# argmaxinc/WhisperKit

Measured on NVIDIA H100. Metric: RTFx (audio-sec/s) whisper-large-v3 greedy, higher is better.
Workload: dtype bf16

## Files before the change

whisperkit_b200/csrc/attention_wgmma.cu:

```cuda
#include <stdio.h>
#include <stdlib.h>

#include "common.cuh"
#include "kernels.h"
#include "wgmma.cuh"

namespace wk {

static constexpr int kFaThreads = 384;
static constexpr int kFaBM = 128;
static constexpr int kFaBN = 128;
static constexpr int kFaD = 64;
static constexpr int kFaTile = kFaBN * kFaD * 2;
static constexpr int kFaStages = 4;
static constexpr int kFaSmem = kFaTile  + 2 * kFaStages * kFaTile  + 1024  + 256 ;

struct FaParams {
    int T, H, dm, n_kv_tiles;
    float scale_log2e;
};

__device__ __forceinline__ float fa_ex2(float x) {
    float y;
    asm("ex2.approx.ftz.f32 %0, %1;" : "=f"(y) : "f"(x));
    return y;
}

template <typename T>
__global__ void __launch_bounds__(kFaThreads, 1)
encoder_attention_wgmma_kernel(const __grid_constant__ CUtensorMap tm_qkv, T* __restrict__ out, const FaParams p) {
    extern __shared__ __align__(1024) uint8_t smem_raw[];
    uint8_t* smem = reinterpret_cast<uint8_t*>((reinterpret_cast<uintptr_t>(smem_raw) + 1023) & ~uintptr_t(1023));
    uint8_t* sQ = smem;
    uint8_t* sK = sQ + kFaTile;
    uint8_t* sV = sK + kFaStages * kFaTile;
    uint64_t* bars = reinterpret_cast<uint64_t*>(sV + kFaStages * kFaTile);
    uint64_t* q_full = bars;
    uint64_t* k_full = bars + 1;
    uint64_t* k_empty = k_full + kFaStages;
    uint64_t* v_full = k_empty + kFaStages;
    uint64_t* v_empty = v_full + kFaStages;

    const int warp = threadIdx.x >> 5, lane = threadIdx.x & 31;
    const int bh = blockIdx.y;
    const int b = bh / p.H, h = bh % p.H;
    const int q0 = blockIdx.x * kFaBM;
    const int n = p.n_kv_tiles;

    if (warp == 0 && lane == 0) {
        tma_prefetch_desc(&tm_qkv);
        mbar_init(q_full, 1);
        for (int i = 0; i < kFaStages; ++i) {
            mbar_init(&k_full[i], 1); mbar_init(&k_empty[i], 8);
            mbar_init(&v_full[i], 1); mbar_init(&v_empty[i], 8);
        }
        fence_barrier_init();
    }
    __syncthreads();

    if (warp < 4) {
        asm volatile("setmaxnreg.dec.sync.aligned.u32 40;");
        if (warp == 0 && lane == 0) {
            mbar_expect_tx(q_full, kFaTile);
            tma_load_3d(sQ, &tm_qkv, q_full, h * kFaD, q0, b);
            for (int j = 0; j < n; ++j) {
                const int st = j % kFaStages;
                const uint32_t ph = (j / kFaStages) & 1;
                mbar_wait_bounded(&k_empty[st], ph ^ 1);
                mbar_expect_tx(&k_full[st], kFaTile);
                tma_load_3d(sK + st * kFaTile, &tm_qkv, &k_full[st], p.dm + h * kFaD, j * kFaBN, b);
                mbar_wait_bounded(&v_empty[st], ph ^ 1);
                mbar_expect_tx(&v_full[st], kFaTile);
                tma_load_3d(sV + st * kFaTile, &tm_qkv, &v_full[st], 2 * p.dm + h * kFaD, j * kFaBN, b);
            }
        }
        return;
    }

    asm volatile("setmaxnreg.inc.sync.aligned.u32 232;");
    const int cw = (warp >> 2) - 1;
    const int c_lo = 2 * (lane & 3);
    const float c = p.scale_log2e;
    const uint64_t qd = wgmma_desc_sw128(smem_u32(sQ + cw * 64 * 128));
    float o[32];
#pragma unroll
    for (int i = 0; i < 32; ++i) o[i] = 0.f;
    float m_run[2] = {-INFINITY, -INFINITY}, l_run[2] = {0.f, 0.f};

    mbar_wait_bounded(q_full, 0);
    for (int j = 0; j < n; ++j) {
        const int st = j % kFaStages;
        const uint32_t ph = (j / kFaStages) & 1;
        float s[64];
        mbar_wait_bounded(&k_full[st], ph);
        const uint64_t kd = wgmma_desc_sw128(smem_u32(sK + st * kFaTile));
        wgmma_fence();
#pragma unroll
        for (int k = 0; k < kFaD / 16; ++k) Wgmma<T, 128>::ss(s, qd + (uint64_t)(2 * k), kd + (uint64_t)(2 * k), k > 0 ? 1u : 0u);
        wgmma_commit();
        wgmma_wait<0>();
        __syncwarp();
        if (lane == 0) mbar_arrive(&k_empty[st]);

        const int valid = p.T - j * kFaBN;
        if (valid < kFaBN) {
#pragma unroll
            for (int jj = 0; jj < 16; ++jj)
#pragma unroll
                for (int e = 0; e < 4; ++e)
                    if (8 * jj + c_lo + (e & 1) >= valid) s[4 * jj + e] = -INFINITY;
        }
        uint32_t pa[8][4];
#pragma unroll
        for (int hf = 0; hf < 2; ++hf) {
            float mx = m_run[hf];
#pragma unroll
            for (int jj = 0; jj < 16; ++jj) mx = fmaxf(mx, fmaxf(s[4 * jj + 2 * hf], s[4 * jj + 2 * hf + 1]));
            mx = fmaxf(mx, __shfl_xor_sync(0xffffffffu, mx, 1));
            mx = fmaxf(mx, __shfl_xor_sync(0xffffffffu, mx, 2));
            const float corr = fa_ex2((m_run[hf] - mx) * c);
            m_run[hf] = mx;
            const float nmc = -mx * c;
            float sum = 0.f;
#pragma unroll
            for (int jj = 0; jj < 16; ++jj) {
                const float e0 = fa_ex2(fmaf(s[4 * jj + 2 * hf], c, nmc));
                const float e1 = fa_ex2(fmaf(s[4 * jj + 2 * hf + 1], c, nmc));
                sum += e0 + e1;
                pa[jj >> 1][(jj & 1) * 2 + hf] = T16<T>::pack2(e0, e1);
            }
            l_run[hf] = l_run[hf] * corr + sum;
#pragma unroll
            for (int jj = 0; jj < 8; ++jj) { o[4 * jj + 2 * hf] *= corr; o[4 * jj + 2 * hf + 1] *= corr; }
        }

        mbar_wait_bounded(&v_full[st], ph);
        const uint32_t vs = smem_u32(sV + st * kFaTile);
        wgmma_fence();
#pragma unroll
        for (int kk = 0; kk < kFaBN / 16; ++kk) Wgmma<T, 64>::rs_bt(o, pa[kk], wgmma_desc_sw128(vs + kk * 2048), 1u);
        wgmma_commit();
        wgmma_wait<0>();
        __syncwarp();
        if (lane == 0) mbar_arrive(&v_empty[st]);
    }

#pragma unroll
    for (int hf = 0; hf < 2; ++hf) {
        float l = l_run[hf];
        l += __shfl_xor_sync(0xffffffffu, l, 1);
        l += __shfl_xor_sync(0xffffffffu, l, 2);
        const float inv = 1.f / l;
        const int q = q0 + cw * 64 + (warp & 3) * 16 + (lane >> 2) + 8 * hf;
        if (q >= p.T) continue;
        T* dst = out + ((long long)b * p.T + q) * p.dm + h * kFaD + c_lo;
#pragma unroll
        for (int jj = 0; jj < 8; ++jj)
            *reinterpret_cast<uint32_t*>(dst + 8 * jj) = T16<T>::pack2(o[4 * jj + 2 * hf] * inv, o[4 * jj + 2 * hf + 1] * inv);
    }
}

typedef CUresult (*PFN_encodeTiled)(CUtensorMap*, CUtensorMapDataType, cuuint32_t, void*, const cuuint64_t*, const cuuint64_t*,
                                      const cuuint32_t*, const cuuint32_t*, CUtensorMapInterleave, CUtensorMapSwizzle,
                                      CUtensorMapL2promotion, CUtensorMapFloatOOBfill);

wk_status encoder_attention_wgmma(const void* qkv, void* out, int B, int T, int n_heads, int dtype, cudaStream_t stream) {
    static PFN_encodeTiled enc = nullptr;
    if (!enc) {
        void* fp = nullptr;
        cudaDriverEntryPointQueryResult q;
        if (cudaGetDriverEntryPoint("cuTensorMapEncodeTiled", &fp, cudaEnableDefault, &q) != cudaSuccess || q != cudaDriverEntryPointSuccess) {
            set_error("cuTensorMapEncodeTiled entry point unavailable");
            return WK_ERR_CUDA;
        }
        enc = reinterpret_cast<PFN_encodeTiled>(fp);
    }
    const int dm = n_heads * 64;
    CUtensorMap tm;
    cuuint64_t gdim[3] = {(cuuint64_t)3 * dm, (cuuint64_t)T, (cuuint64_t)B};
    cuuint64_t gstr[2] = {(cuuint64_t)3 * dm * 2, (cuuint64_t)T * 3 * dm * 2};
    cuuint32_t box[3] = {64, 128, 1};
    cuuint32_t es[3] = {1, 1, 1};
    CUresult r = enc(&tm, dtype == WK_DTYPE_F16 ? CU_TENSOR_MAP_DATA_TYPE_FLOAT16 : CU_TENSOR_MAP_DATA_TYPE_BFLOAT16, 3,
                     const_cast<void*>(qkv), gdim, gstr, box, es, CU_TENSOR_MAP_INTERLEAVE_NONE, CU_TENSOR_MAP_SWIZZLE_128B,
                     CU_TENSOR_MAP_L2_PROMOTION_L2_256B, CU_TENSOR_MAP_FLOAT_OOB_FILL_NONE);
    if (r != CUDA_SUCCESS) { set_error("attention tensor map encode failed: %d", (int)r); return WK_ERR_CUDA; }
    FaParams p;
    p.T = T; p.H = n_heads; p.dm = dm;
    p.n_kv_tiles = (T + kFaBN - 1) / kFaBN;
    p.scale_log2e = 0.125f * 1.4426950408889634f;
    dim3 grid((T + kFaBM - 1) / kFaBM, B * n_heads);
    cudaError_t e = cudaSuccess;
    if (dtype == WK_DTYPE_F16) {
        static bool set = false;
        if (!set) { e = cudaFuncSetAttribute(encoder_attention_wgmma_kernel<__half>, cudaFuncAttributeMaxDynamicSharedMemorySize, kFaSmem); set = e == cudaSuccess; }
        if (e == cudaSuccess) encoder_attention_wgmma_kernel<__half><<<grid, kFaThreads, kFaSmem, stream>>>(tm, (__half*)out, p);
    } else {
        static bool set = false;
        if (!set) { e = cudaFuncSetAttribute(encoder_attention_wgmma_kernel<__nv_bfloat16>, cudaFuncAttributeMaxDynamicSharedMemorySize, kFaSmem); set = e == cudaSuccess; }
        if (e == cudaSuccess) encoder_attention_wgmma_kernel<__nv_bfloat16><<<grid, kFaThreads, kFaSmem, stream>>>(tm, (__nv_bfloat16*)out, p);
    }
    if (e != cudaSuccess) { set_error("cudaFuncSetAttribute(fa): %s", cudaGetErrorString(e)); return WK_ERR_CUDA; }
    count_launch();
    e = cudaGetLastError();
    if (e != cudaSuccess) { set_error("encoder_attention_wgmma launch: %s", cudaGetErrorString(e)); return WK_ERR_CUDA; }
    return WK_OK;
}

}
```

Measured before the change: 919.8.

## Pipeline encoder attention: overlap QK^T with PV and ping-pong warpgroups

Restructures the consumer loop of the wgmma flash-attention kernel so that the S=QK^T GEMM for tile t is issued together with the PV GEMM for tile t-1, and softmax runs while the PV wgmma is still in flight. It also adds named-barrier turn-taking between the two consumer warpgroups so their tensor-core issue phases alternate with each other's softmax phases. The aim is to hide exponential and softmax latency behind tensor-core work. The cost is more live registers (s, pa and o held across iterations), extra named-barrier synchronisation, and more complex pipeline bookkeeping with prologue and epilogue stages.

Measured after the change: 927.8, median of 6. Within noise of the previous version (+0.9%).

```diff
diff --git a/whisperkit_b200/csrc/attention_wgmma.cu b/whisperkit_b200/csrc/attention_wgmma.cu
--- a/whisperkit_b200/csrc/attention_wgmma.cu
+++ b/whisperkit_b200/csrc/attention_wgmma.cu
@@ -20,10 +20,60 @@
     float scale_log2e;
 };
 
+struct FaSlot {
+    int st;
+    uint32_t ph;
+};
+__device__ __forceinline__ FaSlot fa_slot(int j) { return {j % kFaStages, (uint32_t)(j / kFaStages) & 1u}; }
+
+static constexpr int kFaTurnBar = 1;
+__device__ __forceinline__ void fa_turn_wait(int cw) { asm volatile("bar.sync %0, 256;" ::"r"(kFaTurnBar + cw) : "memory"); }
+__device__ __forceinline__ void fa_turn_pass(int cw) { asm volatile("bar.arrive %0, 256;" ::"r"(kFaTurnBar + (cw ^ 1)) : "memory"); }
+
+__device__ __forceinline__ void fa_wait(uint64_t* bar, uint32_t parity) {
+    if (mbar_try_wait(bar, parity)) return;
+    const unsigned long long t0 = globaltimer_ns();
+    unsigned int spins = 0;
+    while (!mbar_try_wait(bar, parity))
+        if ((++spins & 0xfffu) == 0 && globaltimer_ns() - t0 > kSpinLimitNs) __trap();
+}
+
 __device__ __forceinline__ float fa_ex2(float x) {
     float y;
     asm("ex2.approx.ftz.f32 %0, %1;" : "=f"(y) : "f"(x));
     return y;
+}
+
+__device__ __forceinline__ void fa_softmax(float (&s)[64], float (&m_run)[2], float (&l_run)[2], float (&corr)[2], int valid, int c_lo,
+                                           float c) {
+    if (valid < kFaBN) {
+#pragma unroll
+        for (int jj = 0; jj < 16; ++jj)
+#pragma unroll
+            for (int e = 0; e < 4; ++e)
+                if (8 * jj + c_lo + (e & 1) >= valid) s[4 * jj + e] = -INFINITY;
+    }
+#pragma unroll
+    for (int hf = 0; hf < 2; ++hf) {
+        float mx = m_run[hf];
+#pragma unroll
+        for (int jj = 0; jj < 16; ++jj) mx = fmaxf(mx, fmaxf(s[4 * jj + 2 * hf], s[4 * jj + 2 * hf + 1]));
+        mx = fmaxf(mx, __shfl_xor_sync(0xffffffffu, mx, 1));
+        mx = fmaxf(mx, __shfl_xor_sync(0xffffffffu, mx, 2));
+        corr[hf] = fa_ex2((m_run[hf] - mx) * c);
+        m_run[hf] = mx;
+        const float nmc = -mx * c;
+        float sum = 0.f;
+#pragma unroll
+        for (int jj = 0; jj < 16; ++jj) {
+            const float e0 = fa_ex2(fmaf(s[4 * jj + 2 * hf], c, nmc));
+            const float e1 = fa_ex2(fmaf(s[4 * jj + 2 * hf + 1], c, nmc));
+            sum += e0 + e1;
+            s[4 * jj + 2 * hf] = e0;
+            s[4 * jj + 2 * hf + 1] = e1;
+        }
+        l_run[hf] = l_run[hf] * corr[hf] + sum;
+    }
 }
 
 template <typename T>
@@ -64,14 +114,13 @@
             mbar_expect_tx(q_full, kFaTile);
             tma_load_3d(sQ, &tm_qkv, q_full, h * kFaD, q0, b);
             for (int j = 0; j < n; ++j) {
-                const int st = j % kFaStages;
-                const uint32_t ph = (j / kFaStages) & 1;
-                mbar_wait_bounded(&k_empty[st], ph ^ 1);
-                mbar_expect_tx(&k_full[st], kFaTile);
-                tma_load_3d(sK + st * kFaTile, &tm_qkv, &k_full[st], p.dm + h * kFaD, j * kFaBN, b);
-                mbar_wait_bounded(&v_empty[st], ph ^ 1);
-                mbar_expect_tx(&v_full[st], kFaTile);
-                tma_load_3d(sV + st * kFaTile, &tm_qkv, &v_full[st], 2 * p.dm + h * kFaD, j * kFaBN, b);
+                const FaSlot sl = fa_slot(j);
+                fa_wait(&k_empty[sl.st], sl.ph ^ 1);
+                mbar_expect_tx(&k_full[sl.st], kFaTile);
+                tma_load_3d(sK + sl.st * kFaTile, &tm_qkv, &k_full[sl.st], p.dm + h * kFaD, j * kFaBN, b);
+                fa_wait(&v_empty[sl.st], sl.ph ^ 1);
+                mbar_expect_tx(&v_full[sl.st], kFaTile);
+                tma_load_3d(sV + sl.st * kFaTile, &tm_qkv, &v_full[sl.st], 2 * p.dm + h * kFaD, j * kFaBN, b);
             }
         }
         return;
@@ -86,63 +135,81 @@
 #pragma unroll
     for (int i = 0; i < 32; ++i) o[i] = 0.f;
     float m_run[2] = {-INFINITY, -INFINITY}, l_run[2] = {0.f, 0.f};
-
-    mbar_wait_bounded(q_full, 0);
-    for (int j = 0; j < n; ++j) {
-        const int st = j % kFaStages;
-        const uint32_t ph = (j / kFaStages) & 1;
-        float s[64];
-        mbar_wait_bounded(&k_full[st], ph);
+    float s[64];
+    uint32_t pa[8][4];
+
+    const auto issue_s = [&](int st) {
         const uint64_t kd = wgmma_desc_sw128(smem_u32(sK + st * kFaTile));
-        wgmma_fence();
 #pragma unroll
         for (int k = 0; k < kFaD / 16; ++k) Wgmma<T, 128>::ss(s, qd + (uint64_t)(2 * k), kd + (uint64_t)(2 * k), k > 0 ? 1u : 0u);
         wgmma_commit();
-        wgmma_wait<0>();
+    };
+    const auto issue_pv = [&](int st) {
+        const uint32_t vaddr = smem_u32(sV + st * kFaTile);
+#pragma unroll
+        for (int kk = 0; kk < kFaBN / 16; ++kk) Wgmma<T, 64>::rs_bt(o, pa[kk], wgmma_desc_sw128(vaddr + kk * 2048), 1u);
+        wgmma_commit();
+    };
+    const auto release = [&](uint64_t* empty) {
         __syncwarp();
-        if (lane == 0) mbar_arrive(&k_empty[st]);
-
-        const int valid = p.T - j * kFaBN;
-        if (valid < kFaBN) {
-#pragma unroll
-            for (int jj = 0; jj < 16; ++jj)
-#pragma unroll
-                for (int e = 0; e < 4; ++e)
-                    if (8 * jj + c_lo + (e & 1) >= valid) s[4 * jj + e] = -INFINITY;
-        }
-        uint32_t pa[8][4];
-#pragma unroll
-        for (int hf = 0; hf < 2; ++hf) {
-            float mx = m_run[hf];
-#pragma unroll
-            for (int jj = 0; jj < 16; ++jj) mx = fmaxf(mx, fmaxf(s[4 * jj + 2 * hf], s[4 * jj + 2 * hf + 1]));
-            mx = fmaxf(mx, __shfl_xor_sync(0xffffffffu, mx, 1));
-            mx = fmaxf(mx, __shfl_xor_sync(0xffffffffu, mx, 2));
-            const float corr = fa_ex2((m_run[hf] - mx) * c);
-            m_run[hf] = mx;
-            const float nmc = -mx * c;
-            float sum = 0.f;
-#pragma unroll
-            for (int jj = 0; jj < 16; ++jj) {
-                const float e0 = fa_ex2(fmaf(s[4 * jj + 2 * hf], c, nmc));
-                const float e1 = fa_ex2(fmaf(s[4 * jj + 2 * hf + 1], c, nmc));
-                sum += e0 + e1;
-                pa[jj >> 1][(jj & 1) * 2 + hf] = T16<T>::pack2(e0, e1);
-            }
-            l_run[hf] = l_run[hf] * corr + sum;
-#pragma unroll
-            for (int jj = 0; jj < 8; ++jj) { o[4 * jj + 2 * hf] *= corr; o[4 * jj + 2 * hf + 1] *= corr; }
-        }
-
-        mbar_wait_bounded(&v_full[st], ph);
-        const uint32_t vs = smem_u32(sV + st * kFaTile);
+        if (lane == 0) mbar_arrive(empty);
+    };
+    const auto pack_p = [&]() {
+#pragma unroll
+        for (int jj = 0; jj < 16; ++jj)
+#pragma unroll
+            for (int hf = 0; hf < 2; ++hf) pa[jj >> 1][(jj & 1) * 2 + hf] = T16<T>::pack2(s[4 * jj + 2 * hf], s[4 * jj + 2 * hf + 1]);
+    };
+    const auto scale_o = [&](const float (&corr)[2]) {
+#pragma unroll
+        for (int hf = 0; hf < 2; ++hf)
+#pragma unroll
+            for (int jj = 0; jj < 8; ++jj) { o[4 * jj + 2 * hf] *= corr[hf]; o[4 * jj + 2 * hf + 1] *= corr[hf]; }
+    };
+    float corr[2];
+
+    if (cw == 1) fa_turn_pass(cw);
+    fa_wait(q_full, 0);
+    {
+        const FaSlot ks = fa_slot(0);
+        fa_wait(&k_full[ks.st], ks.ph);
+        fa_turn_wait(cw);
         wgmma_fence();
-#pragma unroll
-        for (int kk = 0; kk < kFaBN / 16; ++kk) Wgmma<T, 64>::rs_bt(o, pa[kk], wgmma_desc_sw128(vs + kk * 2048), 1u);
-        wgmma_commit();
-        wgmma_wait<0>();
-        __syncwarp();
-        if (lane == 0) mbar_arrive(&v_empty[st]);
+        issue_s(ks.st);
+        if (cw == 0 || n > 1) fa_turn_pass(cw);
+        wgmma_wait<0>();
+        release(&k_empty[ks.st]);
+        fa_softmax(s, m_run, l_run, corr, p.T, c_lo, c);
+    }
+    for (int t = 1; t < n; ++t) {
+        const FaSlot ks = fa_slot(t), vs = fa_slot(t - 1);
+        fa_turn_wait(cw);
+        wgmma_wait<0>();
+        if (t > 1) release(&v_empty[fa_slot(t - 2).st]);
+        scale_o(corr);
+        pack_p();
+        fa_wait(&k_full[ks.st], ks.ph);
+        fa_wait(&v_full[vs.st], vs.ph);
+        wgmma_fence();
+        issue_s(ks.st);
+        issue_pv(vs.st);
+        if (cw == 0 || t + 1 < n) fa_turn_pass(cw);
+
+        wgmma_wait<1>();
+        release(&k_empty[ks.st]);
+        fa_softmax(s, m_run, l_run, corr, p.T - t * kFaBN, c_lo, c);
+    }
+    {
+        wgmma_wait<0>();
+        if (n > 1) release(&v_empty[fa_slot(n - 2).st]);
+        scale_o(corr);
+        pack_p();
+        const FaSlot vs = fa_slot(n - 1);
+        fa_wait(&v_full[vs.st], vs.ph);
+        wgmma_fence();
+        issue_pv(vs.st);
+        wgmma_wait<0>();
+        release(&v_empty[vs.st]);
     }
 
 #pragma unroll
```
